# AlexandraLJones/MCBRaT3D

Hardware: AMD Instinct MI355X
Metric: photons/sec (higher is better)
Workload: dtype f32/f64

## Files before the change

include/mcbrat.h:

```cpp
#ifndef MCBRAT_H
#define MCBRAT_H
#include <stdint.h>

#ifdef __cplusplus
extern "C" {
#endif

#define MCBRAT_MAX_COMPONENTS 8
#define MCBRAT_MAX_DIRECTIONS 64
#define MCBRAT_ABI_VERSION 3

typedef struct mcbrat_ctx mcbrat_ctx;

typedef struct {
  int32_t fate;
  int32_t ix, iy, iz;
  int32_t nScatter;
  int32_t nEvents;
  float weight;
} mcbrat_fate;

typedef struct {
  int64_t legs, crossings, collisions, absorbEvents, topExits, surfaceHits,
          rouletteKills, rouletteSurvivals;
// ... 34 lines not shown
int mcbrat_specify_intensity(mcbrat_ctx *ctx, int32_t nDirections, const float *intensityMus,
                             const float *intensityPhisDeg, int32_t useRussianRouletteForIntensity,
                             float zetaMin, int32_t useHybridPhaseFunsForIntenCalcs,
                             int32_t numOrdersOrigPhaseFunIntenCalcs,
                             int32_t limitIntensityContributions, float maxIntensityContribution);
int mcbrat_set_forward_table(mcbrat_ctx *ctx, int32_t component, int32_t nAngles, int32_t nEntries,
                             const float *table, const float *origTable);
int mcbrat_report_intensity(mcbrat_ctx *ctx, float *meanIntensity, float *intensity);

int64_t mcbrat_moments_length(const mcbrat_ctx *ctx);
int mcbrat_bind_moments(mcbrat_ctx *ctx, double *deviceBuffer);
double *mcbrat_moments_device_pointer(mcbrat_ctx *ctx);

int mcbrat_frequency_distribution(mcbrat_ctx *ctx, uint64_t seed, uint64_t firstDraw, int32_t numLambda, const double *cdf,
                                  int64_t totalPhotons, int64_t *distribution);
int mcbrat_reset_moments(mcbrat_ctx *ctx);
int mcbrat_get_moments(mcbrat_ctx *ctx, double *hostBuffer);

int mcbrat_enable_counters(mcbrat_ctx *ctx, int32_t enable);
int mcbrat_get_counters(mcbrat_ctx *ctx, mcbrat_counters *out);
const char *mcbrat_first_drop(mcbrat_ctx *ctx);
float mcbrat_last_trace_ms(const mcbrat_ctx *ctx);
int mcbrat_set_async(mcbrat_ctx *ctx, int32_t enable);
int mcbrat_synchronize(mcbrat_ctx *ctx);
int mcbrat_stream_wait_done(mcbrat_ctx *ctx, void *hipStream);
int mcbrat_wait_stream(mcbrat_ctx *ctx, void *hipStream);
int mcbrat_chain_after(mcbrat_ctx *ctx, mcbrat_ctx *previous);
int mcbrat_set_tuning(mcbrat_ctx *ctx, int32_t blocksPerCU, int32_t eventThreshold, int32_t maxBatchesInFlight,
                      int32_t privateTallies, int32_t blockSize, int32_t launchThreshold, int32_t surfaceThreshold,
                      int32_t brickLayout);
// ... 41 lines not shown
```

mcbrat3d_amd/_capi.py:

```python
import ctypes as C
import os
import re

import numpy as np

_HERE = os.path.dirname(os.path.abspath(__file__))
LIB_PATH = os.environ.get("MCBRAT_LIB", os.path.join(_HERE, "libmcbrat_hip.so"))
_lib = None


class McbratError(RuntimeError):
    """A failure status from the integrator (the reference's stateIsFailure(status))."""


class Fate(C.Structure):
    _fields_ = [("fate", C.c_int32), ("ix", C.c_int32), ("iy", C.c_int32), ("iz", C.c_int32),
                ("nScatter", C.c_int32), ("nEvents", C.c_int32), ("weight", C.c_float)]


FATE_DTYPE = np.dtype([("fate", "<i4"), ("ix", "<i4"), ("iy", "<i4"), ("iz", "<i4"),
                       ("nScatter", "<i4"), ("nEvents", "<i4"), ("weight", "<f4")])


class Counters(C.Structure):
# ... 33 lines not shown
    "mcbrat_forward_table_tabulated": (C.c_int, [_i32, _vp, _vp, _i32, _vp]),
    "mcbrat_hybrid_phase_functions": (C.c_int, [_i32, _i32, _vp, _f, _vp]),
    "mcbrat_get_event_threshold": (C.c_int, [_vp]),
    "mcbrat_set_async": (C.c_int, [_vp, _i32]),
    "mcbrat_synchronize": (C.c_int, [_vp]),
    "mcbrat_stream_wait_done": (C.c_int, [_vp, _vp]),
    "mcbrat_wait_stream": (C.c_int, [_vp, _vp]),
    "mcbrat_chain_after": (C.c_int, [_vp, _vp]),
    "mcbrat_set_tuning": (C.c_int, [_vp] + [_i32] * 8),
    "mcbrat_set_walk_options": (C.c_int, [_vp, _i32, _i32]),
    "mcbrat_set_option": (C.c_int, [_vp, C.c_char_p, _i32]),
    "mcbrat_first_drop": (C.c_char_p, [_vp]),
    "mcbrat_get_walk_mode": (C.c_int, [_vp]),
    "mcbrat_moments_device_pointer": (_vp, [_vp]),
    "mcbrat_frequency_distribution": (C.c_int, [_vp, _u64, _u64, _i32, _vp, _i64, _vp]),
    "mcbrat_set_surface_description": (C.c_int, [_vp, _i32, _i32, _vp, _vp, _vp]),
    "mcbrat_trace_fates": (C.c_int, [_vp, _u64, _u64, _i64, _vp]),
    "mcbrat_inverse_table_legendre": (C.c_int, [_i32, _vp, _i32, _vp]),
    "mcbrat_inverse_table_tabulated": (C.c_int, [_i32, _vp, _vp, _i32, _vp]),
    "mcbrat_block_decomposition": (C.c_int, [_i32, _i32, _i32, _vp, _vp, _vp, _vp]),
    "mcbrat_flight_tables": (C.c_int, [_i32, _i32, _i32, _vp, _vp, _vp, _vp, _vp, _vp, _vp]),
    "mcbrat_emission_weighting": (C.c_int, [_i32] * 4 + [_vp] * 7 + [_d] * 4 + [_vp] * 3),
}


ABI_VERSION = 3


def hip_runtimes():
    found = set()
# ... 56 lines not shown
```

mcbrat3d_amd/csrc/mcbrat_api.hip:

```cpp
#include <hip/hip_runtime.h>

#include <algorithm>
#include <cfloat>
#include <cmath>
#include <cstdio>
#include <cstdlib>
#include <cstring>
#include <string>
#include <vector>

#include "mcbrat_kernels.hip"
#include "mcbrat_blockwalk.hip"

using namespace mcbrat;

struct mcbrat_ctx {
  int device = 0;
  struct Lane {
    hipStream_t stream = nullptr;
    hipEvent_t ev0 = nullptr, ev1 = nullptr;
    hipEvent_t evDone = nullptr;
    unsigned long long *dCounter = nullptr;
    long long *dSlabs = nullptr;
    size_t slabCapacity = 0;
// ... 30 lines not shown
  double *dLayerRunT = nullptr;
  float *dExtWalk = nullptr, *dBgVal = nullptr;
  uint16_t *dFlyRange = nullptr;
  int flyNbx = 0, flyNby = 0;
  bool flyBuilt = false;
  double flyDepth = 0.0;
  double flightMaxDepth = 0.5;
  uint32_t *dBlockRec = nullptr;
  uint16_t *dBlockOf = nullptr;
  float *dBlockExt = nullptr;
  float *dBlockSsa = nullptr, *dBlockCum = nullptr;
  uint16_t *dBlockPfi = nullptr;
  bool blockOpticsUniform = false;
  int nBlocks = 0;
  int crossThreshold = 8;
  int jumpThreshold = 8;
  float *dExtB = nullptr, *dCumB = nullptr, *dSsaB = nullptr, *dBgExt = nullptr, *dBgCum = nullptr, *dBgSsa = nullptr;
  uint16_t *dPfiB = nullptr, *dBgPfi = nullptr;
  int nbx = 0, nby = 0, nbz = 0;
  long long nStored = 0;
  double backgroundFraction = 0.0;
  bool bricksBuilt = false;
  int brickMode = 2;
  float *dTables = nullptr;
  int surfNumX = 0, surfNumY = 0;
  double *dSurfX = nullptr, *dSurfY = nullptr;
  float *dSurfRefl = nullptr;
  double *dVoxelCDF = nullptr;
  unsigned long long *dEventCounters = nullptr;
  float *dLast = nullptr;
// ... 585 lines not shown
                              : launch_trace_t<BLOCK, false, 1, false, DBG>(c, p, L.lds, nBatches);
  if (L.brick) return L.tblLds ? launch_trace_t<BLOCK, true, 0, true, DBG>(c, p, L.lds, nBatches)
                               : launch_trace_t<BLOCK, false, 0, true, DBG>(c, p, L.lds, nBatches);
  return L.tblLds ? launch_trace_t<BLOCK, true, 0, false, DBG>(c, p, L.lds, nBatches)
                  : launch_trace_t<BLOCK, false, 0, false, DBG>(c, p, L.lds, nBatches);
}

bool block_walk_applies(const mcbrat_ctx *c, const LaunchPlan &L) {
  return blocks_worth_it(c) && ((L.priv && L.gridLds) || L.blockLite);
}

template <int BLOCK, bool TBL, bool DBG, bool EMIT, int SIMPLE, int OPT = 0>
int launch_block_s(mcbrat_ctx *c, DevParams &p, size_t lds, int nBatches) {
  auto kernel = trace_block_kernel<BLOCK, TBL, DBG, EMIT, SIMPLE, OPT>;
  if (lds + 512 > c->ldsPerCU) return fail(c, "computeRadiativeTransfer: the block-walk tables do not fit the LDS of a compute unit.");
  if (lds > kLdsBudget)
    HIP_OK(c, hipFuncSetAttribute(reinterpret_cast<const void *>(kernel), hipFuncAttributeMaxDynamicSharedMemorySize, (int)lds));
  int perCU = c->blocksPerCU;
  if (perCU <= 0) {
    HIP_OK(c, hipOccupancyMaxActiveBlocksPerMultiprocessor(&perCU, kernel, BLOCK, lds));
    perCU = std::max(1, std::min(perCU, 8));
  }
  unsigned long long blocks = (unsigned long long)perCU * c->numCUs;
  const unsigned long long upb = units_per_batch(blocks, p.ppb, nBatches, BLOCK);
  p.unitsPerBatch = upb;
  p.nUnits = upb * (unsigned long long)nBatches;
  blocks = std::min(blocks, p.nUnits);
  p.ldsBytes = (unsigned)lds;
  hipLaunchKernelGGL(kernel, dim3((unsigned)std::max<unsigned long long>(1, blocks)), dim3(BLOCK), lds, c->L().stream, p);
  HIP_OK(c, hipGetLastError());
  return 0;
}

template <int BLOCK, bool TBL, bool DBG, bool EMIT, int OPT = 0>
int launch_block_e(mcbrat_ctx *c, DevParams &p, size_t lds, int nBatches) {
  const bool simple = c->xyRegular && c->zRegular && c->nc == 1 && c->surfNumX == 0;
  if constexpr (OPT == 0 && BLOCK != 1024) {
    if (simple && c->ny == 1 && !DBG) return launch_block_s<BLOCK, TBL, DBG, EMIT, 2, OPT>(c, p, lds, nBatches);
  }
  if constexpr (!DBG && (BLOCK == 1024 || BLOCK == 768)) {
    if (!c->xyRegular && !c->zRegular && p.xyNearUniform && p.zNearUniform && c->nc == 1 && c->surfNumX == 0 && !getenv("MCBRAT_NO_SIMPLE3"))
      return launch_block_s<BLOCK, TBL, DBG, EMIT, 3, OPT>(c, p, lds, nBatches);
// ... 111 lines not shown
int mcbrat_abi_version(void) { return MCBRAT_ABI_VERSION; }

mcbrat_ctx *mcbrat_create(int device) {
  int n = 0;
  if (hipGetDeviceCount(&n) != hipSuccess || n <= 0 || device < 0 || device >= n) return nullptr;
  if (hipSetDevice(device) != hipSuccess) return nullptr;
  mcbrat_ctx *c = new mcbrat_ctx();
  c->device = device;
  if (const char *e = getenv("MCBRAT_REGULAR_WALK")) c->regularWalk = atoi(e);
  if (const char *e = getenv("MCBRAT_LAYER_SKIP")) c->layerSkip = atoi(e);
  if (const char *e = getenv("MCBRAT_BLOCK_WALK")) c->blockWalk = atoi(e);
  if (const char *e = getenv("MCBRAT_FLIGHT_MAX_DEPTH")) c->flightMaxDepth = atof(e);
  if (const char *e = getenv("MCBRAT_WIDE")) c->wideDefault = c->wideMode = std::max(0, std::min(2, atoi(e)));
  if (const char *e = getenv("MCBRAT_JUMP_THRESHOLD")) c->jumpThreshold = std::max(1, std::min(64, atoi(e)));
  if (const char *e = getenv("MCBRAT_CROSS_THRESHOLD")) c->crossThreshold = std::max(1, std::min(64, atoi(e)));
  if (const char *e = getenv("MCBRAT_RAY_DEFER")) c->rayDefer = atoi(e);
  if (const char *e = getenv("MCBRAT_RAY_SHORT")) c->rayShort = std::max(1, atoi(e));
  if (const char *e = getenv("MCBRAT_RAY_PASS_ITERS")) c->rayPassIters = std::max(1, atoi(e));
  if (const char *e = getenv("MCBRAT_RAY_PASS_AT")) c->rayPassAt = std::max(1, atoi(e));
  if (const char *e = getenv("MCBRAT_TUNE_PHOTONS")) c->tuneTrialPhotons = strtoull(e, nullptr, 10);
  if (const char *e = getenv("MCBRAT_WATCHDOG")) c->watchdog = (unsigned)std::max(16ll, atoll(e));
  if (const char *e = getenv("MCBRAT_MAX_EVENTS")) c->maxEvents = (unsigned)std::max(16ll, atoll(e));
  if (const char *e = getenv("MCBRAT_MAX_EVENTS_NAN")) c->maxEventsNaN = (unsigned)std::max(16ll, atoll(e));
  if (const char *e = getenv("MCBRAT_TEST_LEGACY_TIES")) c->legacyTies = atoi(e);
  if (const char *e = getenv("MCBRAT_TEST_RAY_MAX_LEN")) c->testRayMaxLen = (float)atof(e);
  hipDeviceProp_t prop;
  if (hipGetDeviceProperties(&prop, device) == hipSuccess) {
    c->numCUs = prop.multiProcessorCount;
    if (prop.maxSharedMemoryPerMultiProcessor > 0) c->ldsPerCU = prop.maxSharedMemoryPerMultiProcessor;
  }
// ... 427 lines not shown
    snprintf(buf + at, sizeof(buf) - (size_t)at, "; first recorded: %s in %s, photon id %llu, %s %u, leg %u", kind < 7 ? kinds[kind] : "?",
             kernel == 2 ? "trace_block_kernel" : "trace_kernel", h[3], kind == DROP_RAY ? "view direction" : "state", state, (unsigned)(h[2] >> 32));
  } else {
    snprintf(buf + at, sizeof(buf) - (size_t)at, "; no photon record (production kernels keep none: trace the same photons with mcbrat_trace_fates)");
  }
  c->dropText = buf;
  return c->dropText.c_str();
}

int mcbrat_set_option(mcbrat_ctx *c, const char *name, int32_t value) {
  if (!c) return 1;
  if (!name) return fail(c, "set_option: no option name");
  const std::string n(name);
  if (n == "jumpThreshold") c->jumpThreshold = std::max(1, std::min(64, (int)value));
  else if (n == "crossThreshold") c->crossThreshold = std::max(1, std::min(64, (int)value));
  else return fail(c, "set_option: unknown option '" + n + "'");
  return 0;
}

int mcbrat_set_surface_description(mcbrat_ctx *c, int32_t numX, int32_t numY, const double *xPosition, const double *yPosition,
                                   const float *reflectance) {
  if (!c) return 1;
  (void)hipSetDevice(c->device);
  if (sync_all(c)) return 1;
  if (numX <= 0 || numY <= 0) { c->surfNumX = c->surfNumY = 0; return 0; }
  if (numX < 2 || numY < 2 || !xPosition || !yPosition || !reflectance)
    return fail(c, "new_SurfaceDescription: position vector(s) are incorrect length.");
  for (int i = 1; i < numX; ++i) if (!(xPosition[i] - xPosition[i - 1] > 0.)) return fail(c, "new_SurfaceDescription: positions must be unique, increasing.");
  for (int i = 1; i < numY; ++i) if (!(yPosition[i] - yPosition[i - 1] > 0.)) return fail(c, "new_SurfaceDescription: positions must be unique, increasing.");
  for (size_t i = 0; i < (size_t)(numX - 1) * (numY - 1); ++i)
// ... 41 lines not shown
  unsigned long long *dCounts = c->dFreqCounts;
  HIP_OK(c, hipMemcpyAsync(dCdf, cdf, sizeof(double) * numLambda, hipMemcpyHostToDevice, st));
  HIP_OK(c, hipMemsetAsync(dCounts, 0, sizeof(unsigned long long) * numLambda, st));
  if (totalPhotons > 0) {
    const unsigned long long blocks4 = ((unsigned long long)totalPhotons + 3) / 4 + 1;
    const unsigned grid = (unsigned)std::min<unsigned long long>((blocks4 + 255) / 256, (unsigned long long)c->numCUs * 8);
    const size_t lds = numLambda <= 8192 ? sizeof(unsigned) * (size_t)numLambda : 0;
    hipLaunchKernelGGL(frequency_distribution_kernel, dim3(std::max(1u, grid)), dim3(256), lds, st, dCdf, numLambda,
                       (unsigned long long)totalPhotons, (unsigned long long)firstDraw, (uint32_t)seed, (uint32_t)(seed >> 32), dCounts);
    HIP_OK(c, hipGetLastError());
  }
  std::vector<unsigned long long> h(numLambda);
  HIP_OK(c, hipMemcpyAsync(h.data(), dCounts, sizeof(unsigned long long) * numLambda, hipMemcpyDeviceToHost, st));
  HIP_OK(c, hipStreamSynchronize(st));
  for (int i = 0; i < numLambda; ++i) distribution[i] = (int64_t)h[i];
  return 0;
}

int mcbrat_get_walk_mode(const mcbrat_ctx *c) {
  if (!c) return 0;
  int m = (c->layerSkip ? 1 : 0) | (c->blockWalk ? 2 : 0);
  if (c->haveGrid && c->haveOptics) {
    const size_t ncol = (size_t)c->nx * c->ny;
    LaunchPlan L = plan_launch(c, 2 * ncol + ncol * c->nz);
    if (L.priv && L.brick) { L.priv = false; L.gridLds = false; }
    m = (c->layerSkip ? 1 : 0) | (block_walk_applies(c, L) ? 2 : 0) | (L.fly ? 4 : 0) | (c->blockWalk ? 8 : 0) |
        (L.wide ? 16 : 0) | ((L.blockLite && L.optics == 1) ? 32 : 0) | (L.priv ? 64 : 0) | ((L.blockLite && L.optics == 2) ? 128 : 0) |
        (L.cdfTop ? 256 : 0);
  }
  return m;
// ... 225 lines not shown
```

mcbrat3d_amd/csrc/mcbrat_blockwalk.hip:

```cpp
#include <float.h>

#include "mcbrat_device.h"

namespace mcbrat {

enum : int { BW_DEAD = 0, BW_MOVE = 1, BW_COLLIDE = 2, BW_SURFACE = 3, BW_TOP = 4, BW_CROSS = 5 };

__device__ __forceinline__ int locate_z(const double *ze, int nz, bool regular, double z0, double invDz, double z) {
  if (!regular) return find_cell(ze, nz, z);
  return min(max((int)((z - z0) * invDz), 0), nz - 1);
}
__device__ __forceinline__ int locate_near_uniform(const double *e, int n, double x0, double invCell, double v) {
  int i = min(max((int)((v - x0) * invCell), 0), n - 1);
  const double lo = e[i], hi = e[i + 1];
  i += (v >= hi && i < n - 1) ? 1 : 0;
  i -= (v < lo && i > 0) ? 1 : 0;
  return i;
}

__device__ __forceinline__ long long unwrapped_index(const double *e, int n, double x0, double L, double invL, double x) {
  const double k = floor((x - x0) * invL);
  return (long long)k * n + find_cell(e, n, x - k * L);
}

// ... 28 lines not shown
  constexpr bool NOY = SIMPLE == 2 && !DEBUG;
  constexpr bool NEAR = SIMPLE == 3;
  const bool xyRegular = NEAR ? false : (SIMPLE != 0 ? true : p.xyRegular != 0);
  const bool zRegular = NEAR ? false : (SIMPLE != 0 ? true : p.zRegular != 0);
  const int nc = SIMPLE != 0 ? 1 : p.nc;
  extern __shared__ __align__(16) unsigned char smem_raw[];
#ifdef MCBRAT_POISON
  for (unsigned i = threadIdx.x; i < p.ldsBytes / 4u; i += BLOCK) reinterpret_cast<unsigned *>(smem_raw)[i] = 0xffffffffu;
  __syncthreads();
#endif
  double *s_edge = reinterpret_cast<double *>(smem_raw);
  const int nEdges = p.nx + p.ny + p.nz + 3;
  const int ncol = p.nx * p.ny;
  const int nvox = ncol * p.nz;
  const int slabLen = (int)p.slabStride;
  const bool cdfTop = EMIT && p.cdfTopLds != 0;
  const BlockLds lay = block_lds_layout(p.nx, p.ny, p.nz, nc, (size_t)slabLen, p.nBlocks, TBL_LDS ? (size_t)p.tblTotalFloats : 0, OPT, cdfTop);
  const int nB4 = (p.nBlocks + 3) & ~3;
  long long *s_slab = reinterpret_cast<long long *>(smem_raw + lay.slab);
  unsigned *s_cursor = reinterpret_cast<unsigned *>(smem_raw + lay.cursor);
  uint4 *s_blockRec = reinterpret_cast<uint4 *>(smem_raw + lay.rec);
  float *s_ext = reinterpret_cast<float *>(smem_raw + lay.ext);
  double *s_cdfLevel = reinterpret_cast<double *>(smem_raw + lay.cdf);
  double *s_cdfRow = s_cdfLevel + p.nz;
  float *s_ssa = reinterpret_cast<float *>(smem_raw + lay.ssa);
  float *s_cum = reinterpret_cast<float *>(smem_raw + lay.cum);
  uint16_t *s_pfi = reinterpret_cast<uint16_t *>(smem_raw + lay.pfi);
  uint16_t *s_blockOf = reinterpret_cast<uint16_t *>(smem_raw + lay.blockOf);
  float *s_tbl = reinterpret_cast<float *>(smem_raw + lay.tbl);
  __shared__ int s_tblOffset[MCBRAT_MAX_COMPONENTS], s_tblNSteps[MCBRAT_MAX_COMPONENTS];
  __shared__ float s_tblInvN[MCBRAT_MAX_COMPONENTS];
  if (threadIdx.x < MCBRAT_MAX_COMPONENTS) {
    s_tblOffset[threadIdx.x] = p.tblOffset[threadIdx.x];
    s_tblNSteps[threadIdx.x] = p.tblNSteps[threadIdx.x];
    s_tblInvN[threadIdx.x] = p.tblInvN[threadIdx.x];
  }
  for (int i = threadIdx.x; i < nEdges; i += BLOCK) s_edge[i] = p.edges[i];
  if (TBL_LDS)
    for (int i = threadIdx.x; i < p.tblTotalFloats; i += BLOCK) s_tbl[i] = p.tables[i];
  for (int i = threadIdx.x; i < slabLen; i += BLOCK) s_slab[i] = 0;
  if (threadIdx.x == 0) s_cursor[0] = 0;
  for (int i = threadIdx.x; i < p.nBlocks; i += BLOCK) s_blockRec[i] = p.blockRec[i];
  for (int i = threadIdx.x; i < nvox; i += BLOCK) s_blockOf[i] = p.blockOf[i];
  if (OPT == 0) {
    for (int i = threadIdx.x; i < nvox; i += BLOCK) s_ext[i] = p.ext[i];
    for (int i = threadIdx.x; i < nc * nvox; i += BLOCK) { s_ssa[i] = p.ssa[i]; s_pfi[i] = p.pfi[i]; }
    if (nc > 1)
      for (int i = threadIdx.x; i < nc * nvox; i += BLOCK) s_cum[i] = p.cum[i];
  } else {
    for (int i = threadIdx.x; i < p.nBlocks; i += BLOCK) s_ext[i] = p.blockExt[i];
    if (OPT == 2) {
      for (int i = threadIdx.x; i < nc * nB4; i += BLOCK) {
        const int k = i / nB4, b = i - k * nB4;
        if (b < p.nBlocks) { s_ssa[i] = p.blockSsa[k * p.nBlocks + b]; s_pfi[i] = p.blockPfi[k * p.nBlocks + b]; if (nc > 1) s_cum[i] = p.blockCum[k * p.nBlocks + b]; }
      }
// ... 5 lines not shown
    for (int i = threadIdx.x; i < p.ny * p.nz; i += BLOCK) { const int k = i / p.ny, j = i - k * p.ny; s_cdfRow[i] = p.voxelCDF[((long long)p.nx - 1) + (long long)p.nx * j + nxy * k]; }
  }
  __syncthreads();
  auto cumAt = [&](int k, int cell) -> float { if constexpr (OPT == 0) return s_cum[k * nvox + cell]; else if constexpr (OPT == 1) return p.cum[k * nvox + cell]; else return s_cum[k * nB4 + s_blockOf[cell]]; };
  auto ssaAt = [&](int k, int cell) -> float { if constexpr (OPT == 0) return s_ssa[k * nvox + cell]; else if constexpr (OPT == 1) return p.ssa[k * nvox + cell]; else return s_ssa[k * nB4 + s_blockOf[cell]]; };
  auto pfiAt = [&](int k, int cell) -> int { if constexpr (OPT == 0) return (int)s_pfi[k * nvox + cell]; else if constexpr (OPT == 1) return (int)p.pfi[k * nvox + cell]; else return (int)s_pfi[k * nB4 + s_blockOf[cell]]; };
  auto extOfCell = [&](int cell) -> float { if constexpr (OPT == 0) return s_ext[cell]; else return s_ext[s_blockOf[cell]]; };
  const float *__restrict__ tbl = TBL_LDS ? s_tbl : p.tables;
  const int offY = p.nx + 1, offZ = p.nx + p.ny + 2;
  const double invDz = (double)p.nz / (p.zMax - p.z0);

  const int lane = threadIdx.x & (kWave - 1);
  const unsigned long long laneBelow = (1ull << lane) - 1ull;

  unsigned long long unitFirst = 0;
  unsigned unitCount = 0;
  long long *unitSlab = nullptr;

  int state = BW_DEAD;
  bool more = true;
  uint32_t idLo = 0, idHi = 0, event = 0;
  double px = 0, py = 0, pz = 0;
  float dx = 0, dy = 0, dz = 1;
  float ivx = 0, ivy = 0, ivz = 0;
  float tnx = 0, tny = 0, tnz = 0, tcur = 0;
  float acc = 0, tau = 0, w = 0, extCur = 0, uX = 0, uY = 0, uZ = 0;
  unsigned rx = 0, ry = 0, rz = 0;
  unsigned spans = 0;
  int nScat = 0, nLegs = 0;
  long long dbgX = 0, dbgY = 0;
  int dbgZ = 0;
  unsigned int cLegs = 0, cCross = 0, cColl = 0, cAbs = 0, cTop = 0, cSurf = 0, cKill = 0, cSurv = 0;
  unsigned long long wIters = 0, wCrossPhases = 0, wCrossLanes = 0, wEventLanes = 0, wLaunchPhases = 0, wSurfPhases = 0;

  auto countCrossings = [&](double x, double y, int kzEnd) {
// ... 49 lines not shown
  unsigned nBadLane = 0;
  const unsigned maxEvents = (DEBUG || kTestBounds) ? p.maxEvents : kMaxEvents, maxEventsNaN = (DEBUG || kTestBounds) ? p.maxEventsNaN : kMaxEventsNaN,
                 watchdog = (DEBUG || kTestBounds) ? p.watchdog : kWatchdog;
#define MCBRAT_BW_DROP(kind_) do { \
    if constexpr (DEBUG || kTestBounds) record_first_drop(p.bad, (kind_), 2u, idLo, idHi, state, event);   \
    if (DEBUG && p.fates) p.fates[(((unsigned long long)idHi << 32) | idLo) - p.firstPhoton] = mcbrat_fate{3, 0, 0, 0, nScat, nLegs, w}; \
    state = BW_DEAD; \
    nBadLane = count_drop(nBadLane, (kind_));   \
  } while (0)
#ifdef MCBRAT_STAMPS
  __shared__ unsigned long long s_tprev[BLOCK / 64], s_stamp[BLOCK / 64][9];
  if (lane == 0) { s_tprev[threadIdx.x >> 6] = clock64(); for (int i = 0; i < 9; i++) s_stamp[threadIdx.x >> 6][i] = 0; }
#endif
  for (unsigned long long unit = blockIdx.x;; unit += gridDim.x) {
    if (unit >= p.nUnits) break;
    uint32_t batch;
    {
      const unsigned long long b = unit / p.unitsPerBatch, s = unit % p.unitsPerBatch;
      const unsigned long long bp = (p.total - b * p.ppb) < p.ppb ? (p.total - b * p.ppb) : p.ppb;
      const unsigned long long lo = (bp * s) / p.unitsPerBatch, hi = (bp * (s + 1)) / p.unitsPerBatch;
      unitFirst = b * p.ppb + lo;
      unitCount = (unsigned)(hi - lo);
      unitSlab = p.slabs + b * p.slabStride;
      batch = (uint32_t)b;
      more = true;
    }
    (void)batch;

    for (;;) {
      bool needLeg = false;
      int ix = 0, iy = 0, iz = 0;

      const unsigned long long mSurf = __ballot(state == BW_SURFACE || state == BW_TOP);
      const unsigned long long mCross = __ballot(state == BW_CROSS);
      const int nBusy = __popcll(__ballot(state == BW_COLLIDE));
      const bool idle = nBusy < p.eventThreshold;
      const bool doSurface = __popcll(mSurf) >= p.surfaceThreshold || idle;
      const bool doCross = __popcll(mCross) >= p.crossThreshold || idle;
      if ((state == BW_SURFACE || state == BW_TOP) && doSurface) {
        const bool top = state == BW_TOP;
        {
          const double xw = px + (double)tcur * (double)dx, yw = py + (double)tcur * (double)dy;
// ... 6 lines not shown
            const double lo = s_edge[rx & 0xffffu], hi = s_edge[rx >> 16];
            if (px < lo && lo - px > px + p.Lx - hi) px += p.Lx;
            else if (px > hi && px - hi > lo - (px - p.Lx)) px -= p.Lx;
          }
          iy = 0;
          if (!NOY) {
            const int jy = locY(yw, true, true);
            iy = inRange(jy, ry);
            if (iy != jy) {
              const double lo = s_edge[offY + (ry & 0xffffu)], hi = s_edge[offY + (ry >> 16)];
              if (py < lo && lo - py > py + p.Ly - hi) py += p.Ly;
              else if (py > hi && py - hi > lo - (py - p.Ly)) py -= p.Ly;
            }
          }
        }
        atomicAdd(reinterpret_cast<unsigned long long *>(s_slab + (top ? 0 : ncol) + (ix + p.nx * iy)), weight_to_fixed(w));
        if (top) {
          if (DEBUG) {
            cTop++;
            if (p.fates) p.fates[(((unsigned long long)idHi << 32) | idLo) - p.firstPhoton] = mcbrat_fate{0, ix + 1, iy + 1, p.nz + 1, nScat, nLegs, w};
          }
          state = BW_DEAD;
        } else {
          pz = p.zSurf;
          iz = 0;
          nScat++;
          if (DEBUG) cSurf++;
          float mu = sqrtf(uX);
          if (!(fabsf(mu) > 2.0f * FLT_MIN)) {
            mu = sqrtf(uZ);
            uint32_t r[4];
// ... 30 lines not shown
      }
      if (want != 0ull) {
        const int nWant = __popcll(want);
        const int rank = __popcll(want & laneBelow);
        unsigned base = 0;
        if (lane == 0) base = atomicAdd(&s_cursor[0], (unsigned)nWant);
        base = (unsigned)__shfl((int)base, 0);
        const unsigned k = base + (unsigned)rank;
        const bool valid = k < unitCount;
        const unsigned long long myIdx = unitFirst + k;
        if (state == BW_DEAD && more) {
          if (valid) {
            const unsigned long long id = p.firstPhoton + myIdx;
            idLo = (uint32_t)id; idHi = (uint32_t)(id >> 32);
            event = 0; nScat = 0; nLegs = 0;
            uint32_t r[4];
            philox4x32_10(0u, 0u, idLo, idHi, p.seedLo, p.seedHi, r);
            double lx, ly, lz;
            if (!EMIT) {
              lx = (double)u01(r[0]);
              ly = (double)u01(r[1]);
              lz = 0.0;
              dx = p.dir0[0]; dy = p.dir0[1]; dz = p.dir0[2];
            } else {
              float mu = 0.f, phi = 0.f;
              const float sel = u01(r[0]);
              if ((double)sel > p.fracAtms) {
                lx = (double)u01(r[1]);
                ly = (double)u01(r[2]);
                lz = 0.0;
// ... 43 lines not shown
              ix = NEAR ? locate_near_uniform(s_edge, p.nx, p.x0, p.invCellX, px) : find_cell(s_edge, p.nx, px);
              iy = NOY ? 0 : (NEAR ? locate_near_uniform(s_edge + offY, p.ny, p.y0, p.invCellY, py) : find_cell(s_edge + offY, p.ny, py));
            }
            if (!EMIT) {
              pz = p.zLaunch; iz = p.izLaunch;
            } else if (zRegular) {
              pz = p.z0 + lz * (p.zMax - p.z0);
              iz = min((int)((pz - p.z0) / ((p.zMax - p.z0) / (double)p.nz)), p.nz - 1);
            } else {
              const double t = (lz - p.z0) * (double)p.nz;
              const double fl = floor(t);
              iz = min((int)fl, p.nz - 1);
              pz = s_edge[offZ + iz] + (t - fl) * (s_edge[offZ + iz + 1] - s_edge[offZ + iz]);
            }
            if (EMIT && p.lwFlag && pz > 0.0)
              atomicAdd(reinterpret_cast<unsigned long long *>(s_slab + 2 * ncol + (ix + p.nx * (iy + p.ny * iz))), to_fixed(-1.0));
            needLeg = true;
          } else {
            more = false;
          }
        }
      }
      STAMP(0);
      if (state == BW_COLLIDE) {
        if (dz == dz || legacyMoveNaN) {
          const double s = (double)(tcur + div_fast(tau - acc, extCur));
          px = px + s * (double)dx;
          if (!NOY) py = py + s * (double)dy;
          pz = pz + s * (double)dz;
        }
        {
// ... 14 lines not shown
        int pfEntry = pfiAt(c, cell);
        if (ssa <= 0.0f && extOfCell(cell) != extCur) {
          ix = inRange(ix, rx); iz = inRange(iz, rz);
          if (!NOY) iy = inRange(iy, ry);
          cell = ix + p.nx * (iy + p.ny * iz);
          c = 0;
          if (nc > 1) {
            for (int k = 0; k < nc - 1; k++)
              if (uZ >= cumAt(k, cell)) c = k + 1;
          }
          ssa = ssaAt(c, cell);
          pfEntry = pfiAt(c, cell);
        }
        if (DEBUG) countCrossings(px, py, iz);
        if (ssa < 1.0f) {
          atomicAdd(reinterpret_cast<unsigned long long *>(s_slab + 2 * ncol + cell), weight_to_fixed(w * (1.0f - ssa)));
          w = w * ssa;
          if (DEBUG) cAbs++;
        }
        if (p.useRR && w < 0.5f) {
          float uR = uZ;
          if (nc != 1) {
            uint32_t r1[4];
            philox4x32_10(event, 1u, idLo, idHi, p.seedLo, p.seedHi, r1);
            uR = u01(r1[1]);
          }
          if (uR >= w) { w = 0.0f; if (DEBUG) cKill++; }
          else { w = 1.0f; if (DEBUG) cSurv++; }
        }
        STAMP(2);
        if (w <= FLT_MIN) {
// ... 124 lines not shown
        if (accNew > tau) {
          state = BW_COLLIDE;
        } else if (!(tmin < FLT_MAX)) {
          MCBRAT_BW_DROP(DROP_VACUUM);
        } else {
          acc = accNew;
          tcur = tmin;
          state = BW_CROSS;
          if (isZ && (dz >= 0.0f ? (int)(rz >> 16) == p.nz : (rz & 0xffffu) == 0u)) state = dz >= 0.0f ? BW_TOP : BW_SURFACE;
        }
      }
      STAMP(7);
    }

    __syncthreads();
    for (int i = threadIdx.x; i < slabLen; i += BLOCK) {
      const long long v = s_slab[i];
      if (v != 0) {
        atomicAdd(reinterpret_cast<unsigned long long *>(unitSlab + i), (unsigned long long)v);
        s_slab[i] = 0;
      }
    }
    if (threadIdx.x == 0) s_cursor[0] = 0;
    __syncthreads();
  }

  publish_drops(p.bad, nBadLane);
#ifdef MCBRAT_STAMPS
  if (DEBUG && p.counters && lane == 0) for (int i = 0; i < 9; i++) atomicAdd(p.counters + 16 + i, s_stamp[threadIdx.x >> 6][i]);
#endif
  if (DEBUG && p.counters) {
// ... 18 lines not shown
```

mcbrat3d_amd/csrc/mcbrat_device.h:

```cpp
#pragma once
#include <hip/hip_runtime.h>
#include <stdint.h>

#include "../../include/mcbrat.h"

namespace mcbrat {

constexpr int kWave = 64;
constexpr double kTallyScale = 4294967296.0;
constexpr double kTallyInv = 1.0 / 4294967296.0;

constexpr unsigned kMaxEvents = 1u << 24;
constexpr unsigned kMaxEventsNaN = 1u << 20;
constexpr unsigned kWatchdog = 1u << 20;

#ifdef MCBRAT_TEST_BOUNDS_IN_PRODUCTION
constexpr bool kTestBounds = true;
#else
constexpr bool kTestBounds = false;
#endif

enum : unsigned { DROP_LEGS = 1, DROP_NAN_LEGS = 2, DROP_WATCHDOG = 3, DROP_CROSSINGS = 4, DROP_VACUUM = 5, DROP_RAY = 6 };
constexpr int kBadWords = 8;
constexpr unsigned kBadCountMask = 0x03ffffffu;
// ... 79 lines not shown
  int useRRIntensity;
  float zetaMin;
  int rayShort, rayPassIters, rayPassAt;
  int rayCap;
  int limitContrib;
  float maxContrib;
  unsigned long long *counter;
  unsigned long long total;
  unsigned long long ppb;
  unsigned long long firstPhoton;
  uint32_t seedLo, seedHi;
  long long *slabs;
  unsigned long long slabStride;
  unsigned long long nUnits;
  unsigned long long unitsPerBatch;
  int eventThreshold;
  int launchThreshold;
  int surfaceThreshold;
  int jumpThreshold;
  unsigned long long *bad;
  unsigned maxEvents;
  unsigned maxEventsNaN;
  unsigned watchdog;
  float rayMaxLen;
  int legacyTies;
  unsigned ldsBytes;
  mcbrat_fate *fates;
  unsigned long long *counters;
  double *traceBuf;
  unsigned long long traceIndex;
// ... 5 lines not shown
```

mcbrat3d_amd/csrc/mcbrat_kernels.hip:

```cpp
#include <float.h>

#include "mcbrat_device.h"

#ifdef MCBRAT_STAMPS
#define STAMP(i) do { if (DEBUG && p.counters) { const unsigned long long t_ = clock64(); \
    if (lane == __ffsll((long long)__ballot(1)) - 1) { s_stamp[threadIdx.x >> 6][i] += t_ - s_tprev[threadIdx.x >> 6]; s_tprev[threadIdx.x >> 6] = t_; } } } while (0)
#elif defined(MCBRAT_MARKS)
#define STAMP(i) asm volatile("; @@mark " #i)
#else
#define STAMP(i) do { } while (0)
#endif

namespace mcbrat {

constexpr unsigned kChunk = 256;
#ifndef MCBRAT_FLY_MIN_BRICKS
#define MCBRAT_FLY_MIN_BRICKS 8.0f
#endif
constexpr float kFlyMinBricks = MCBRAT_FLY_MIN_BRICKS;
constexpr int kWalkCap = 256;

#ifndef MCBRAT_MIN_WAVES_PER_SIMD
#define MCBRAT_MIN_WAVES_PER_SIMD 4
#endif
#ifndef MCBRAT_WAVES_GLOBAL_GRID
#define MCBRAT_WAVES_GLOBAL_GRID 6
#endif
#ifndef MCBRAT_WAVES_GLOBAL_GRID_INTEN
#define MCBRAT_WAVES_GLOBAL_GRID_INTEN 4
#endif

__device__ __forceinline__ void philox4x32_10(uint32_t c0, uint32_t c1, uint32_t c2, uint32_t c3, uint32_t k0,
                                              uint32_t k1, uint32_t (&out)[4]) {
#pragma unroll
  for (int i = 0; i < 10; i++) {
    const unsigned long long p0 = (unsigned long long)0xD2511F53u * c0;
    const unsigned long long p1 = (unsigned long long)0xCD9E8D57u * c2;
    c0 = (uint32_t)(p1 >> 32) ^ c1 ^ k0;
    c1 = (uint32_t)p1;
    c2 = (uint32_t)(p0 >> 32) ^ c3 ^ k1;
    c3 = (uint32_t)p0;
    k0 += 0x9E3779B9u;
    k1 += 0xBB67AE85u;
  }
  out[0] = c0; out[1] = c1; out[2] = c2; out[3] = c3;
}

__device__ __forceinline__ float u01(uint32_t u) { return (float)u * 2.3283064365386963e-10f; }

#ifdef MCBRAT_PRECISE_MATH
__device__ __forceinline__ float rcp_fast(float x) { return 1.0f / x; }
__device__ __forceinline__ float div_fast(float a, float b) { return a / b; }
#else
__device__ __forceinline__ float rcp_fast(float x) { return __builtin_amdgcn_rcpf(x); }
__device__ __forceinline__ float div_fast(float a, float b) { return a * __builtin_amdgcn_rcpf(b); }
// ... 1182 lines not shown
    atomicAdd(p.counters + 1, (unsigned long long)cCross);
    atomicAdd(p.counters + 2, (unsigned long long)cColl);
    atomicAdd(p.counters + 3, (unsigned long long)cAbs);
    atomicAdd(p.counters + 4, (unsigned long long)cTop);
    atomicAdd(p.counters + 5, (unsigned long long)cSurf);
    atomicAdd(p.counters + 6, (unsigned long long)cKill);
    atomicAdd(p.counters + 7, (unsigned long long)cSurv);
    if (lane == 0) {
      atomicAdd(p.counters + 8, wWalkIters); atomicAdd(p.counters + 9, wWalkLanes);
      atomicAdd(p.counters + 10, wEventPhases); atomicAdd(p.counters + 11, wEventLanes);
      atomicAdd(p.counters + 12, wLaunchPhases); atomicAdd(p.counters + 13, wSurfPhases);
    }
  }
}

__global__ void frequency_distribution_kernel(const double *cdf, int n, unsigned long long total, unsigned long long firstDraw,
                                              uint32_t seedLo, uint32_t seedHi, unsigned long long *counts) {
  extern __shared__ unsigned int s_hist[];
  const bool useLds = n <= 8192;
  if (useLds) {
    for (int i = threadIdx.x; i < n; i += blockDim.x) s_hist[i] = 0u;
    __syncthreads();
  }
  const unsigned long long nBlocks4 = (firstDraw + total + 3) / 4 - firstDraw / 4;
  for (unsigned long long j = (unsigned long long)blockIdx.x * blockDim.x + threadIdx.x; j < nBlocks4;
       j += (unsigned long long)gridDim.x * blockDim.x) {
    const unsigned long long blk = firstDraw / 4 + j;
    uint32_t r[4];
    philox4x32_10(0xFFFFFFFFu, 0u, (uint32_t)blk, (uint32_t)(blk >> 32), seedLo, seedHi, r);
#pragma unroll
// ... 246 lines not shown
```

Baseline: 5.170 billion.

## Spread block-walk work units across batch boundaries and use bitop3 in Philox

Adds a 'wide units' mode to the block-walk kernel. Photons are split evenly over all resident blocks, ignoring batch boundaries. Each unit keeps two LDS tally slabs, so a unit that spans two batches can flush into both batch slabs. This is meant to remove load imbalance and tail underuse when the per-batch unit count is uneven, at the cost of doubled slab LDS and a larger flush. Philox's triple XOR is fused into one gfx950 bitop3 instruction, and a standalone Philox test kernel and API are added.

```diff
diff --git a/include/mcbrat.h b/include/mcbrat.h
--- a/include/mcbrat.h
+++ b/include/mcbrat.h
@@ -72,6 +72,7 @@
 
 int mcbrat_frequency_distribution(mcbrat_ctx *ctx, uint64_t seed, uint64_t firstDraw, int32_t numLambda, const double *cdf,
                                   int64_t totalPhotons, int64_t *distribution);
+int mcbrat_philox4x32_10(mcbrat_ctx *ctx, int32_t n, const uint32_t *in, uint32_t *out);
 int mcbrat_reset_moments(mcbrat_ctx *ctx);
 int mcbrat_get_moments(mcbrat_ctx *ctx, double *hostBuffer);
 
diff --git a/mcbrat3d_amd/_capi.py b/mcbrat3d_amd/_capi.py
--- a/mcbrat3d_amd/_capi.py
+++ b/mcbrat3d_amd/_capi.py
@@ -71,6 +71,7 @@
     "mcbrat_get_walk_mode": (C.c_int, [_vp]),
     "mcbrat_moments_device_pointer": (_vp, [_vp]),
     "mcbrat_frequency_distribution": (C.c_int, [_vp, _u64, _u64, _i32, _vp, _i64, _vp]),
+    "mcbrat_philox4x32_10": (C.c_int, [_vp, _i32, _vp, _vp]),
     "mcbrat_set_surface_description": (C.c_int, [_vp, _i32, _i32, _vp, _vp, _vp]),
     "mcbrat_trace_fates": (C.c_int, [_vp, _u64, _u64, _i64, _vp]),
     "mcbrat_inverse_table_legendre": (C.c_int, [_i32, _vp, _i32, _vp]),
diff --git a/mcbrat3d_amd/csrc/mcbrat_api.hip b/mcbrat3d_amd/csrc/mcbrat_api.hip
--- a/mcbrat3d_amd/csrc/mcbrat_api.hip
+++ b/mcbrat3d_amd/csrc/mcbrat_api.hip
@@ -68,6 +68,7 @@
   bool blockOpticsUniform = false;
   int nBlocks = 0;
   int crossThreshold = 8;
+  int batchUnits = 0;
   int jumpThreshold = 8;
   float *dExtB = nullptr, *dCumB = nullptr, *dSsaB = nullptr, *dBgExt = nullptr, *dBgCum = nullptr, *dBgSsa = nullptr;
   uint16_t *dPfiB = nullptr, *dBgPfi = nullptr;
@@ -683,18 +684,29 @@
 int launch_block_s(mcbrat_ctx *c, DevParams &p, size_t lds, int nBatches) {
   auto kernel = trace_block_kernel<BLOCK, TBL, DBG, EMIT, SIMPLE, OPT>;
   if (lds + 512 > c->ldsPerCU) return fail(c, "computeRadiativeTransfer: the block-walk tables do not fit the LDS of a compute unit.");
+  int perCU = c->blocksPerCU;
+  if (perCU <= 0) {
+    if (lds > kLdsBudget)
+      HIP_OK(c, hipFuncSetAttribute(reinterpret_cast<const void *>(kernel), hipFuncAttributeMaxDynamicSharedMemorySize, (int)lds));
+    HIP_OK(c, hipOccupancyMaxActiveBlocksPerMultiprocessor(&perCU, kernel, BLOCK, lds));
+    perCU = std::max(1, std::min(perCU, 8));
+  }
+  unsigned long long blocks = (unsigned long long)perCU * c->numCUs;
+  const size_t lds2 = block_lds_layout(p.nx, p.ny, p.nz, SIMPLE != 0 ? 1 : p.nc, 2 * (size_t)p.slabStride, p.nBlocks, TBL ? (size_t)p.tblTotalFloats : 0,
+                                       OPT, EMIT && p.cdfTopLds != 0).total;
+  const unsigned long long units = std::max<unsigned long long>(1, std::min(blocks, p.total));
+  p.unitsWide = !c->batchUnits && (p.total + units - 1) / units <= p.ppb && (size_t)perCU * (lds2 + 512) <= c->ldsPerCU;
+  if (p.unitsWide) {
+    lds = lds2;
+    p.nUnits = blocks = units;
+  } else {
+    const unsigned long long upb = units_per_batch(blocks, p.ppb, nBatches, BLOCK);
+    p.unitsPerBatch = upb;
+    p.nUnits = upb * (unsigned long long)nBatches;
+    blocks = std::min(blocks, p.nUnits);
+  }
   if (lds > kLdsBudget)
     HIP_OK(c, hipFuncSetAttribute(reinterpret_cast<const void *>(kernel), hipFuncAttributeMaxDynamicSharedMemorySize, (int)lds));
-  int perCU = c->blocksPerCU;
-  if (perCU <= 0) {
-    HIP_OK(c, hipOccupancyMaxActiveBlocksPerMultiprocessor(&perCU, kernel, BLOCK, lds));
-    perCU = std::max(1, std::min(perCU, 8));
-  }
-  unsigned long long blocks = (unsigned long long)perCU * c->numCUs;
-  const unsigned long long upb = units_per_batch(blocks, p.ppb, nBatches, BLOCK);
-  p.unitsPerBatch = upb;
-  p.nUnits = upb * (unsigned long long)nBatches;
-  blocks = std::min(blocks, p.nUnits);
   p.ldsBytes = (unsigned)lds;
   hipLaunchKernelGGL(kernel, dim3((unsigned)std::max<unsigned long long>(1, blocks)), dim3(BLOCK), lds, c->L().stream, p);
   HIP_OK(c, hipGetLastError());
@@ -836,6 +848,7 @@
   if (const char *e = getenv("MCBRAT_WIDE")) c->wideDefault = c->wideMode = std::max(0, std::min(2, atoi(e)));
   if (const char *e = getenv("MCBRAT_JUMP_THRESHOLD")) c->jumpThreshold = std::max(1, std::min(64, atoi(e)));
   if (const char *e = getenv("MCBRAT_CROSS_THRESHOLD")) c->crossThreshold = std::max(1, std::min(64, atoi(e)));
+  if (const char *e = getenv("MCBRAT_BATCH_UNITS")) c->batchUnits = atoi(e) != 0;
   if (const char *e = getenv("MCBRAT_RAY_DEFER")) c->rayDefer = atoi(e);
   if (const char *e = getenv("MCBRAT_RAY_SHORT")) c->rayShort = std::max(1, atoi(e));
   if (const char *e = getenv("MCBRAT_RAY_PASS_ITERS")) c->rayPassIters = std::max(1, atoi(e));
@@ -1293,6 +1306,7 @@
   const std::string n(name);
   if (n == "jumpThreshold") c->jumpThreshold = std::max(1, std::min(64, (int)value));
   else if (n == "crossThreshold") c->crossThreshold = std::max(1, std::min(64, (int)value));
+  else if (n == "batchUnits") c->batchUnits = value != 0;
   else return fail(c, "set_option: unknown option '" + n + "'");
   return 0;
 }
@@ -1364,6 +1378,28 @@
   HIP_OK(c, hipMemcpyAsync(h.data(), dCounts, sizeof(unsigned long long) * numLambda, hipMemcpyDeviceToHost, st));
   HIP_OK(c, hipStreamSynchronize(st));
   for (int i = 0; i < numLambda; ++i) distribution[i] = (int64_t)h[i];
+  return 0;
+}
+
+int mcbrat_philox4x32_10(mcbrat_ctx *c, int32_t n, const uint32_t *in, uint32_t *out) {
+  if (!c) return 1;
+  if (n < 0 || (n > 0 && (!in || !out))) return fail(c, "philox4x32_10: invalid arguments.");
+  if (n == 0) return 0;
+  (void)hipSetDevice(c->device);
+  if (init_lane(c, 0)) return 1;
+  hipStream_t st = c->lane[0].stream;
+  uint32_t *dIn = nullptr, *dOut = nullptr;
+  HIP_OK(c, dev_malloc((void **)&dIn, sizeof(uint32_t) * 6 * (size_t)n));
+  if (dev_malloc((void **)&dOut, sizeof(uint32_t) * 4 * (size_t)n) != hipSuccess) { (void)hipFree(dIn); return fail(c, "philox4x32_10: out of device memory."); }
+  hipError_t e = hipMemcpyAsync(dIn, in, sizeof(uint32_t) * 6 * (size_t)n, hipMemcpyHostToDevice, st);
+  if (e == hipSuccess) {
+    hipLaunchKernelGGL(philox_kernel, dim3((unsigned)((n + 255) / 256)), dim3(256), 0, st, dIn, (int)n, dOut);
+    e = hipGetLastError();
+  }
+  if (e == hipSuccess) e = hipMemcpyAsync(out, dOut, sizeof(uint32_t) * 4 * (size_t)n, hipMemcpyDeviceToHost, st);
+  if (e == hipSuccess) e = hipStreamSynchronize(st);
+  (void)hipFree(dIn); (void)hipFree(dOut);
+  HIP_OK(c, e);
   return 0;
 }
 
diff --git a/mcbrat3d_amd/csrc/mcbrat_blockwalk.hip b/mcbrat3d_amd/csrc/mcbrat_blockwalk.hip
--- a/mcbrat3d_amd/csrc/mcbrat_blockwalk.hip
+++ b/mcbrat3d_amd/csrc/mcbrat_blockwalk.hip
@@ -66,8 +66,9 @@
   const int ncol = p.nx * p.ny;
   const int nvox = ncol * p.nz;
   const int slabLen = (int)p.slabStride;
+  const int slabsLen = p.unitsWide ? 2 * slabLen : slabLen;
   const bool cdfTop = EMIT && p.cdfTopLds != 0;
-  const BlockLds lay = block_lds_layout(p.nx, p.ny, p.nz, nc, (size_t)slabLen, p.nBlocks, TBL_LDS ? (size_t)p.tblTotalFloats : 0, OPT, cdfTop);
+  const BlockLds lay = block_lds_layout(p.nx, p.ny, p.nz, nc, (size_t)slabsLen, p.nBlocks, TBL_LDS ? (size_t)p.tblTotalFloats : 0, OPT, cdfTop);
   const int nB4 = (p.nBlocks + 3) & ~3;
   long long *s_slab = reinterpret_cast<long long *>(smem_raw + lay.slab);
   unsigned *s_cursor = reinterpret_cast<unsigned *>(smem_raw + lay.cursor);
@@ -90,7 +91,7 @@
   for (int i = threadIdx.x; i < nEdges; i += BLOCK) s_edge[i] = p.edges[i];
   if (TBL_LDS)
     for (int i = threadIdx.x; i < p.tblTotalFloats; i += BLOCK) s_tbl[i] = p.tables[i];
-  for (int i = threadIdx.x; i < slabLen; i += BLOCK) s_slab[i] = 0;
+  for (int i = threadIdx.x; i < slabsLen; i += BLOCK) s_slab[i] = 0;
   if (threadIdx.x == 0) s_cursor[0] = 0;
   for (int i = threadIdx.x; i < p.nBlocks; i += BLOCK) s_blockRec[i] = p.blockRec[i];
   for (int i = threadIdx.x; i < nvox; i += BLOCK) s_blockOf[i] = p.blockOf[i];
@@ -126,11 +127,12 @@
   const unsigned long long laneBelow = (1ull << lane) - 1ull;
 
   unsigned long long unitFirst = 0;
-  unsigned unitCount = 0;
+  unsigned unitCount = 0, unitSplit = 0;
   long long *unitSlab = nullptr;
 
   int state = BW_DEAD;
   bool more = true;
+  int slabOff = 0;
   uint32_t idLo = 0, idHi = 0, event = 0;
   double px = 0, py = 0, pz = 0;
   float dx = 0, dy = 0, dz = 1;
@@ -210,18 +212,23 @@
 #endif
   for (unsigned long long unit = blockIdx.x;; unit += gridDim.x) {
     if (unit >= p.nUnits) break;
-    uint32_t batch;
-    {
+    if (p.unitsWide) {
+      const unsigned long long lo = p.total * unit / p.nUnits, hi = p.total * (unit + 1) / p.nUnits;
+      const unsigned long long b = lo / p.ppb, end = (b + 1) * p.ppb;
+      unitFirst = lo;
+      unitCount = (unsigned)(hi - lo);
+      unitSplit = (unsigned)((hi < end ? hi : end) - lo);
+      unitSlab = p.slabs + b * p.slabStride;
+    } else {
       const unsigned long long b = unit / p.unitsPerBatch, s = unit % p.unitsPerBatch;
       const unsigned long long bp = (p.total - b * p.ppb) < p.ppb ? (p.total - b * p.ppb) : p.ppb;
       const unsigned long long lo = (bp * s) / p.unitsPerBatch, hi = (bp * (s + 1)) / p.unitsPerBatch;
       unitFirst = b * p.ppb + lo;
       unitCount = (unsigned)(hi - lo);
+      unitSplit = unitCount;
       unitSlab = p.slabs + b * p.slabStride;
-      batch = (uint32_t)b;
-      more = true;
     }
-    (void)batch;
+    more = true;
 
     for (;;) {
       bool needLeg = false;
@@ -258,7 +265,7 @@
             }
           }
         }
-        atomicAdd(reinterpret_cast<unsigned long long *>(s_slab + (top ? 0 : ncol) + (ix + p.nx * iy)), weight_to_fixed(w));
+        atomicAdd(reinterpret_cast<unsigned long long *>(s_slab + slabOff + (top ? 0 : ncol) + (ix + p.nx * iy)), weight_to_fixed(w));
         if (top) {
           if (DEBUG) {
             cTop++;
@@ -319,6 +326,7 @@
             const unsigned long long id = p.firstPhoton + myIdx;
             idLo = (uint32_t)id; idHi = (uint32_t)(id >> 32);
             event = 0; nScat = 0; nLegs = 0;
+            slabOff = k < unitSplit ? 0 : slabLen;
             uint32_t r[4];
             philox4x32_10(0u, 0u, idLo, idHi, p.seedLo, p.seedHi, r);
             double lx, ly, lz;
@@ -392,7 +400,7 @@
               pz = s_edge[offZ + iz] + (t - fl) * (s_edge[offZ + iz + 1] - s_edge[offZ + iz]);
             }
             if (EMIT && p.lwFlag && pz > 0.0)
-              atomicAdd(reinterpret_cast<unsigned long long *>(s_slab + 2 * ncol + (ix + p.nx * (iy + p.ny * iz))), to_fixed(-1.0));
+              atomicAdd(reinterpret_cast<unsigned long long *>(s_slab + slabOff + 2 * ncol + (ix + p.nx * (iy + p.ny * iz))), to_fixed(-1.0));
             needLeg = true;
           } else {
             more = false;
@@ -437,7 +445,7 @@
         }
         if (DEBUG) countCrossings(px, py, iz);
         if (ssa < 1.0f) {
-          atomicAdd(reinterpret_cast<unsigned long long *>(s_slab + 2 * ncol + cell), weight_to_fixed(w * (1.0f - ssa)));
+          atomicAdd(reinterpret_cast<unsigned long long *>(s_slab + slabOff + 2 * ncol + cell), weight_to_fixed(w * (1.0f - ssa)));
           w = w * ssa;
           if (DEBUG) cAbs++;
         }
@@ -592,7 +600,7 @@
     }
 
     __syncthreads();
-    for (int i = threadIdx.x; i < slabLen; i += BLOCK) {
+    for (int i = threadIdx.x; i < slabsLen; i += BLOCK) {
       const long long v = s_slab[i];
       if (v != 0) {
         atomicAdd(reinterpret_cast<unsigned long long *>(unitSlab + i), (unsigned long long)v);
diff --git a/mcbrat3d_amd/csrc/mcbrat_device.h b/mcbrat3d_amd/csrc/mcbrat_device.h
--- a/mcbrat3d_amd/csrc/mcbrat_device.h
+++ b/mcbrat3d_amd/csrc/mcbrat_device.h
@@ -117,6 +117,7 @@
   unsigned long long slabStride;
   unsigned long long nUnits;
   unsigned long long unitsPerBatch;
+  int unitsWide;
   int eventThreshold;
   int launchThreshold;
   int surfaceThreshold;
diff --git a/mcbrat3d_amd/csrc/mcbrat_kernels.hip b/mcbrat3d_amd/csrc/mcbrat_kernels.hip
--- a/mcbrat3d_amd/csrc/mcbrat_kernels.hip
+++ b/mcbrat3d_amd/csrc/mcbrat_kernels.hip
@@ -30,15 +30,23 @@
 #define MCBRAT_WAVES_GLOBAL_GRID_INTEN 4
 #endif
 
+__device__ __forceinline__ uint32_t xor3(uint32_t a, uint32_t b, uint32_t c) {
+#if defined(__gfx950__)
+  return __builtin_amdgcn_bitop3_b32(a, b, c, 0x96);
+#else
+  return a ^ b ^ c;
+#endif
+}
+
 __device__ __forceinline__ void philox4x32_10(uint32_t c0, uint32_t c1, uint32_t c2, uint32_t c3, uint32_t k0,
                                               uint32_t k1, uint32_t (&out)[4]) {
 #pragma unroll
   for (int i = 0; i < 10; i++) {
     const unsigned long long p0 = (unsigned long long)0xD2511F53u * c0;
     const unsigned long long p1 = (unsigned long long)0xCD9E8D57u * c2;
-    c0 = (uint32_t)(p1 >> 32) ^ c1 ^ k0;
+    c0 = xor3((uint32_t)(p1 >> 32), c1, k0);
     c1 = (uint32_t)p1;
-    c2 = (uint32_t)(p0 >> 32) ^ c3 ^ k1;
+    c2 = xor3((uint32_t)(p0 >> 32), c3, k1);
     c3 = (uint32_t)p0;
     k0 += 0x9E3779B9u;
     k1 += 0xBB67AE85u;
@@ -1251,6 +1259,15 @@
   }
 }
 
+__global__ void philox_kernel(const uint32_t *in, int n, uint32_t *out) {
+  const int i = blockIdx.x * blockDim.x + threadIdx.x;
+  if (i >= n) return;
+  const uint32_t *a = in + 6 * (size_t)i;
+  uint32_t r[4];
+  philox4x32_10(a[0], a[1], a[2], a[3], a[4], a[5], r);
+  for (int e = 0; e < 4; ++e) out[4 * (size_t)i + e] = r[e];
+}
+
 __global__ void frequency_distribution_kernel(const double *cdf, int n, unsigned long long total, unsigned long long firstDraw,
                                               uint32_t seedLo, uint32_t seedHi, unsigned long long *counts) {
   extern __shared__ unsigned int s_hist[];
```

Measured after the change: 5.560 billion, median of 6. +7.5%, better.
